# schmeing/ReSeq

Hardware: AMD Instinct MI355X
Metric: simulated read-pairs/sec (2x150 bp) (higher is better)
Workload: dtype f64

## Files before the change

### reseq_amd/csrc/rsq_core.h

```cpp
#pragma once
#include "rsq_types.h"
#if !defined(__HIPCC_RTC__)
#include <math.h>
#endif

namespace rsq {

struct Words {
    uint32_t w0, w1, w2, w3;
};


RSQ_HD Words philox(uint64_t seed, uint32_t c0, uint32_t c1, uint32_t c2, uint32_t c3) {
    uint32_t k0 = (uint32_t)seed, k1 = (uint32_t)(seed >> 32);
#pragma unroll
    for (int r = 0; r < 10; ++r) {
        const uint64_t p0 = (uint64_t)0xD2511F53u * c0, p1 = (uint64_t)0xCD9E8D57u * c2;
        const uint32_t hi0 = (uint32_t)(p0 >> 32), lo0 = (uint32_t)p0, hi1 = (uint32_t)(p1 >> 32), lo1 = (uint32_t)p1;
        c0 = hi1 ^ c1 ^ k0;
        c1 = lo1;
        c2 = hi0 ^ c3 ^ k1;
        c3 = lo0;
        k0 += 0x9E3779B9u;
        k1 += 0xBB67AE85u;
// ... 269 lines not shown
template <int NM, class Par0>
RSQ_HD uint32_t draw(const DevTable &t, const double *__restrict__ pool, Par0 par0, const uint32_t (&idx)[NM], double u, double &prob_sum) {
    prob_sum = 0.0;
    if (!t.k) return 0;
    const uint32_t kp = row_stride(t.k);
    GlobalRow m[NM];
#pragma unroll
    for (int n = 0; n < NM; ++n) m[n].p = pool + t.off[n] + (size_t)clamp_row(t, n, idx[n]) * kp;
    uint32_t col;
    if constexpr (NM == 3) col = draw_rows_k(t.k, u, prob_sum, m[0], m[1], m[2]);
    else col = draw_rows_k(t.k, u, prob_sum, m[0], m[1], m[2], m[3]);
    return par0[t.par0_off + col];
}

template <int NM, class Par0>
RSQ_HD uint32_t draw_slim(const DevTable &t, const double *__restrict__ pool, Par0 par0, const uint32_t (&idx)[NM], double u, double &prob_sum) {
    prob_sum = 0.0;
    if (!t.k) return 0;
    const uint32_t kp = row_stride(t.k);
    GlobalRow m[NM];
#pragma unroll
    for (int n = 0; n < NM; ++n) m[n].p = pool + t.off[n] + (size_t)clamp_row(t, n, idx[n]) * kp;
    uint32_t col;
    if constexpr (NM == 3) col = draw_rows<1>(t.k, u, prob_sum, m[0], m[1], m[2]);
    else col = draw_rows<1>(t.k, u, prob_sum, m[0], m[1], m[2], m[3]);
    return par0[t.par0_off + col];
}

struct GlobalTables {
    using Sum = double;
    const DevSim &S;
    RSQ_HD const DevTable &quality(uint32_t i) const { return S.quality[i]; }
    RSQ_HD const DevTable &seq_quality(uint32_t i) const { return S.seq_quality[i]; }
    RSQ_HD uint32_t draw_quality(uint32_t i, const uint32_t (&idx)[4], uint32_t word, double &ps) const { return draw<4>(S.quality[i], S.pool, S.par0, idx, u32_to_unit(word), ps); }
    RSQ_HD uint32_t draw_base_call(uint32_t i, const uint32_t (&idx)[4], uint32_t word, double &ps) const { return draw<4>(S.base_call[i], S.pool, S.par0, idx, u32_to_unit(word), ps); }
    RSQ_HD uint32_t draw_indel(uint32_t i, const uint32_t (&idx)[3], uint32_t word, double &ps) const { return draw<3>(S.indels[i], S.pool, S.par0, idx, u32_to_unit(word), ps); }
    RSQ_HD uint32_t draw_seq_quality(uint32_t i, const uint32_t (&idx)[3], uint32_t word, double &ps) const { return draw<3>(S.seq_quality[i], S.pool, S.par0, idx, u32_to_unit(word), ps); }
};

RSQ_HD uint32_t ref_base(const uint64_t *__restrict__ words, uint64_t word_off, uint32_t pos) {
    return (uint32_t)(words[word_off + (pos >> 5)] >> ((pos & 31u) * 2u)) & 3u;
}
RSQ_HD uint32_t ref_gc_count(const uint64_t *__restrict__ words, uint64_t word_off, uint32_t a, uint32_t b) {
    uint32_t gc = 0;
    const uint64_t kLow = 0x5555555555555555ull;
    for (uint32_t w = a >> 5; w <= ((b - 1) >> 5) && a < b; ++w) {
        uint64_t x = words[word_off + w];
        uint64_t g = (x ^ (x >> 1)) & kLow;
        uint32_t lo = w == (a >> 5) ? (a & 31u) : 0u;
        uint32_t hi = w == ((b - 1) >> 5) ? ((b - 1) & 31u) + 1u : 32u;
        if (lo) g &= ~0ull << (2u * lo);
        if (hi < 32u) g &= (1ull << (2u * hi)) - 1ull;
#if defined(__HIP_DEVICE_COMPILE__)
        gc += (uint32_t)__popcll(g);
#else
        gc += (uint32_t)__builtin_popcountll(g);
#endif
    }
    return gc;
}

RSQ_HD uint32_t gc_low(uint64_t x, uint32_t n_bases) {
    const uint64_t g = (x ^ (x >> 1)) & 0x5555555555555555ull & ((1ull << (2u * n_bases)) - 1ull);
#if defined(__HIP_DEVICE_COMPILE__)
    return (uint32_t)__popcll(g);
#else
    return (uint32_t)__builtin_popcountll(g);
#endif
// ... 135 lines not shown
    uint32_t seq_qual, qual, error_rate, num_errors;
    uint32_t last_written_qual;
    uint32_t iteration;
};

RSQ_HD uint32_t draw_read_length(const DevSim &S, uint32_t seg, uint32_t fragment_length, double u) {
    const DevReadLengths &rl = S.read_lengths[seg];
    if (rl.fixed) return rl.fixed;
    const double random_value = u * (double)S.insert_lengths[fragment_length];
    double counter = 0.0;
    const uint32_t row = fragment_length - rl.row_first;
    const uint32_t from = rl.row_from[row] & 0xFFFFu;
    uint32_t read_len = (from + (rl.row_ptr[row + 1] - rl.row_ptr[row])) & 0xFFFFu;
    while (counter <= random_value) {
        const bool more = read_len > from;
        read_len = (read_len - 1u) & 0xFFFFu;
        if (!more) break;
        counter += (double)rl.values[rl.row_ptr[row] + (read_len - from)];
    }
    return read_len;
}

template <class Src>
RSQ_HD void template_totals_loop(const Src &src, uint32_t n, uint32_t &gc, uint32_t &rate_sum) {
    for (uint32_t k = 0; k < n; ++k) {
        if (is_gc(src.base(k))) ++gc;
        rate_sum += src.sys_base(k) >> 8;
    }
}

struct AdapterSrc {
    const uint8_t *seq;
    const uint16_t *sys_;
    RSQ_HD uint32_t base(uint32_t k) const { return seq[k]; }
    RSQ_HD uint32_t sys_base(uint32_t k) const { return sys_[k]; }
    RSQ_HD uint32_t sys_deleted(uint32_t k) const { return sys_[k]; }
};

struct ReadMachine {
    enum : uint32_t { kTemplate = 0, kAdapter = 1, kTail = 2, kDone = 3 };
    FillState par;
    CigarRun cg;
    uint32_t phase, seg, tile_id, tbase;
    uint32_t org_pos, org_len;
    uint32_t adapter_id, adapter_a0;
    uint32_t iter_m, hard_clip, tail_length, pos_tail, n_indels;
    uint32_t start_cut_word;

    RSQ_HD void idle() {
        par = FillState{};
        cg = CigarRun{'M', 0, 0};
        phase = kDone;
        seg = tile_id = tbase = org_pos = org_len = adapter_id = adapter_a0 = iter_m = hard_clip = tail_length = pos_tail = n_indels = start_cut_word = 0;
    }
    template <class Tab, class Src>
    RSQ_HD void init(const DevSim &S, const Tab &tab, const Stream &st, uint32_t seg_, uint32_t tile, uint32_t fragment_length, const Src &src) {
        seg = seg_;
        tile_id = tile;
        tbase = (seg * RSQ_SIM(S, n_tiles) + tile_id) * 4u;
        par.read_pos = 0;
        par.previous_indel_type = 0;
        par.indel_pos = 0;
        par.base_call = 5;
        par.gc_seq = 0;
        par.qual = 1;
        par.error_rate = 0;
// ... 63 lines not shown
                org_pos = adapter_pos;
                tail_length = discrete_draw(S.polya_cp, S.polya_n, u32_to_unit(h1.w0)) + S.polya_from;
                cg.element = 'S';
                cg.length = 0;
                phase = kAdapter;
            } else if (phase == kAdapter) {
                if (par.read_pos < par.read_length && org_pos < org_len) return true;
                if (cg.length) cg.flush();
                if (!(par.read_pos < par.read_length)) {
                    phase = kDone;
                    return false;
                }
                hard_clip = par.read_length - par.read_pos;
                cg.chars += digits10(hard_clip) + 1u;
                pos_tail = 0;
                phase = kTail;
            } else if (phase == kTail) {
                if (par.read_pos < par.read_length) return true;
                phase = kDone;
                return false;
            } else return false;
        }
    }

    template <class Tab, class Src, class Out>
    RSQ_HD bool step(const DevSim &S, const Tab &tab, const Stream &st, const Src &src, Out &out) {
        if (!advance(S, st)) return false;
        iterate(S, tab, st, src, out);
        return true;
    }
    RSQ_HD bool in_template() const { return phase == kTemplate && par.read_pos < par.read_length && org_pos < org_len; }
    template <bool TEMPLATE_PART = false, class Tab, class Src, class Out>
    RSQ_HD void iterate(const DevSim &S, const Tab &tab, const Stream &st, const Src &src, Out &out) {
        const bool tail = !TEMPLATE_PART && phase == kTail, from_template = TEMPLATE_PART || phase == kTemplate;
        const DevAdapters &ad = S.adapters[seg];
        const uint32_t it = par.iteration;
        const Words w = st.step(2u + it);
        typename Tab::Sum prob_sum;
        uint32_t indel = 0, org_base = 0;
        if (!tail) {
            const uint32_t idx_i[3] = {par.indel_pos, par.read_pos, par.gc_seq};
            indel = tab.draw_indel(par.previous_indel_type * 6u + par.base_call, idx_i, w.w0, prob_sum);
            if (0 == prob_sum) indel = 0;
            org_base = from_template ? src.base(org_pos) : (uint32_t)ad.seqs[adapter_a0 + org_pos];
        }
        const uint32_t qi = tbase + org_base;
        const bool regular = !tail && 0 == indel, deletion = !tail && 1 == indel;
        uint32_t dom_error = 0;
        if (regular) {
            const uint32_t se = from_template ? src.sys_base(org_pos) : (uint32_t)ad.sys[adapter_a0 + org_pos];
            dom_error = se & 0xFFu;
            par.error_rate = se >> 8;
        } else if (deletion) {
            par.error_rate = (from_template ? src.sys_deleted(org_pos) : (uint32_t)ad.sys[adapter_a0 + org_pos]) >> 8;
        }
        uint32_t q = 0;
        if (!deletion) {
            const uint32_t idx_q[4] = {par.seq_qual, par.qual, par.read_pos, par.error_rate};
            q = tab.draw_quality(qi, idx_q, w.w1, prob_sum);
            if (0 == prob_sum) {
                if (regular) q = par.read_pos ? par.last_written_qual : tab.quality(qi).max_value;
                else if (tail) q = par.read_pos ? par.last_written_qual : q;
                else q = par.qual;
            }
        }
        uint32_t put_base = 0, op_code = 0;
// ... 15 lines not shown
            par.qual = q;
            put_base = pos_tail < tail_length ? 0u : discrete_draw(S.overrun_cp, 4, u32_to_unit(w.w3));
            ++pos_tail;
        } else {
            put_base = indel - 2u;
            op_code = 2u;
            element = 'I';
        }
        if (element) {
            const uint32_t is_indel = deletion || insertion ? 1u : 0u;
            n_indels += is_indel;
            par.num_errors += is_indel;
            if (element == cg.element) {
                ++cg.length;
                par.indel_pos += is_indel;
            } else {
                cg.flush();
                cg.element = element;
                cg.length = 1;
                par.indel_pos = is_indel;
                par.previous_indel_type = deletion ? 1u : 0u;
            }
            if (!insertion) ++org_pos;
        }
        if (!deletion) {
            out.put(par.read_pos, put_base, q + RSQ_SIM(S, phred_offset));
            par.last_written_qual = q;
            ++par.read_pos;
        }
        if (!tail) out.op(it, op_code);
        par.iteration = it + 1u;
    }

    RSQ_HD void finalize(ReadMeta &meta) const {
        meta.read_len = (uint16_t)par.read_length;
        meta.num_errors = (uint16_t)par.num_errors;
        meta.n_iter_m = (uint16_t)iter_m;
        meta.n_iter_s = (uint16_t)(par.iteration - iter_m - hard_clip);
        meta.hard_clip = (uint16_t)hard_clip;
        meta.tile_id = (uint16_t)tile_id;
        meta.cigar_chars = (uint16_t)cg.chars;
        meta.plain = n_indels ? 0u : 1u;
    }
};

template <class Tab, class Src, class Out>
RSQ_HD void fill_read(const DevSim &S, const Tab &tab, const Stream &st, uint32_t seg, uint32_t tile_id, uint32_t fragment_length, const Src &src, Out &out,
                      ReadMeta &meta) {
    ReadMachine m;
    m.init(S, tab, st, seg, tile_id, fragment_length, src);
    while (m.step(S, tab, st, src, out)) {}
    m.finalize(meta);
}

}
```

### reseq_amd/csrc/rsq_reads.h

```cpp
#pragma once
#include "rsq_core.h"
#include "rsq_variants.h"
#include "rsq_text.h"

namespace rsq {

struct ReadOut {
    WordColumn seq, qual, ops;
    uint32_t cur_word, cur_index;
    uint32_t seq_word, qual_word, n_put;
    RSQ_HD void put(uint32_t pos, uint32_t base, uint32_t qual_char) {
        const uint32_t sh = (pos & 3u) * 8u;
        seq_word |= base << sh;
        qual_word |= qual_char << sh;
        n_put = pos + 1u;
        if ((pos & 3u) == 3u) {
            seq.at(pos >> 2) = seq_word;
            qual.at(pos >> 2) = qual_word;
            seq_word = qual_word = 0;
        }
    }
    RSQ_HD void op(uint32_t it, uint32_t code) {
        const uint32_t wi = it >> 4;
        if (wi != cur_index) {
            ops.at(cur_index) = cur_word;
            cur_word = 0;
            cur_index = wi;
        }
        cur_word |= code << ((it & 15u) * 2u);
    }
    RSQ_HD void finish() {
        ops.at(cur_index) = cur_word;
        if (n_put & 3u) {
            seq.at(n_put >> 2) = seq_word;
            qual.at(n_put >> 2) = qual_word;
        }
    }
};
RSQ_HD ReadOut make_read_out(const WordColumn &seq, const WordColumn &qual, const WordColumn &ops) { return ReadOut{seq, qual, ops, 0u, 0u, 0u, 0u, 0u}; }

struct RawLayout {
    uint32_t *seq, *qual;
    uint32_t *ops;
    ReadMeta *meta;
    uint64_t pitch;
    uint64_t *templates;
    uint32_t template_words;
    const uint32_t *order;
    RSQ_HD uint64_t item_of(uint64_t row) const { return order ? order[row] : row; }
    RSQ_HD WordColumn seq_of(uint64_t r) const { return WordColumn{seq + r, pitch}; }
    RSQ_HD WordColumn qual_of(uint64_t r) const { return WordColumn{qual + r, pitch}; }
    RSQ_HD WordColumn ops_of(uint64_t r) const { return WordColumn{ops + r, pitch}; }
    RSQ_HD ReadOut out_of(uint64_t r) const { return make_read_out(seq_of(r), qual_of(r), ops_of(r)); }
};

struct FragmentSrc {
    const uint64_t *words;
    uint64_t word_off;
    uint32_t first;
    uint32_t len;
    bool reverse;
    const uint16_t *sys_;
    const uint64_t *converted;
    const uint32_t *gc_prefix;
    mutable uint32_t held_word = 0xFFFFFFFFu, held_sys = 0xFFFFFFFFu;
    mutable uint64_t word = 0, sys4 = 0;
    RSQ_HD uint64_t template_word(const uint64_t *from, uint32_t index) const {
        if (index != held_word) {
            held_word = index;
            word = from[index];
        }
        return word;
    }
    RSQ_HD uint32_t org_len() const { return len; }
    RSQ_HD uint32_t ref(uint32_t k) const {
        const uint32_t pos = reverse ? first - 1u - k : first + k, b = (uint32_t)(template_word(words + word_off, pos >> 5) >> ((pos & 31u) * 2u)) & 3u;
        return reverse ? 3u - b : b;
    }
    RSQ_HD uint32_t base(uint32_t k) const { return converted ? (uint32_t)(template_word(converted, k >> 5) >> ((k & 31u) * 2u)) & 3u : ref(k); }
    RSQ_HD uint32_t sys_base(uint32_t k) const {
        if ((k >> 2) != held_sys) {
            held_sys = k >> 2;
#if defined(__HIP_DEVICE_COMPILE__)
            sys4 = *reinterpret_cast<const uint64_t __attribute__((aligned(2))) *>(sys_ + (k & ~3u));
#else
            memcpy(&sys4, sys_ + (k & ~3u), 8);
#endif
        }
        return (uint32_t)(sys4 >> ((k & 3u) * 16u)) & 0xFFFFu;
    }
    RSQ_HD uint32_t sys_deleted(uint32_t k) const { return sys_base(k); }
    RSQ_HD void totals(uint32_t n, uint32_t &gc, uint32_t &rate_sum) const {
        if (!converted && !gc_prefix) return template_totals_loop(*this, n, gc, rate_sum);
        if (converted) gc += ref_gc_count(converted, 0, 0, n);
        else gc += reverse ? ref_gc_count_prefix(words, gc_prefix, word_off, first - n, first) : ref_gc_count_prefix(words, gc_prefix, word_off, first, first + n);
        rate_sum += rate_total(n);
    }
// ... 138 lines not shown
                        ++t;
                        continue;
                    }
                    left = side.len(var);
                }
            }
            uint32_t run;
            if (left) {
                run = left < length - t ? left : length - t;
                left -= run;
                if (!left) {
                    var = side.next(var);
                    ++x;
                }
            } else {
                int64_t until = out;
                if (side.variant(var) && side.at(var) > x && side.at(var) < until) until = side.at(var);
                run = until - x < (int64_t)(length - t) ? (uint32_t)(until - x) : length - t;
                x += run;
            }
            ct_convert_run(tmpl, t, run, rate, d);
            t = (uint16_t)(t + run);
        }
        region = side.next(region);
        if (side.region(region) && side.entry(region) > x) skip_to(region);
    }
}
RSQ_HD void ct_conversion(uint64_t *tmpl, uint32_t length, const MethView &m, const VarView *r, uint32_t allele, uint32_t start_pos, bool reversed, VarStart from, MethDraws &d) {
    if (reversed) methylation_walk<true>(tmpl, length, m, r, allele, start_pos, from, d);
    else methylation_walk<false>(tmpl, length, m, r, allele, start_pos, from, d);
}

struct EmptySrc {
    RSQ_HD void totals(uint32_t, uint32_t &, uint32_t &) const {}
    RSQ_HD uint32_t org_len() const { return 0; }
    RSQ_HD uint32_t base(uint32_t) const { return 0; }
    RSQ_HD uint32_t sys_base(uint32_t) const { return 0; }
    RSQ_HD uint32_t sys_deleted(uint32_t) const { return 0; }
};

RSQ_HD uint32_t draw_tile(const DevSim &S, uint32_t c0, uint32_t c1, uint32_t c2, uint32_t c3base) {
    if (RSQ_SIM(S, n_tiles) > 1) return discrete_draw(S.tile_cp, RSQ_SIM(S, n_tiles), u32_to_unit(philox(S.seed, c0, c1, c2, c3base).w0));
    return 0;
}

RSQ_HD uint32_t lds_desc_count(uint32_t n_tiles) { return 25u * n_tiles + 12u; }
RSQ_HD uint32_t image_qbase(const DevSim &S, uint32_t seg, uint32_t first_tile) { return (seg * RSQ_SIM(S, n_tiles) + first_tile) * 4u; }
constexpr uint32_t kDescWords = sizeof(DevTable) / 4u;

#if defined(__HIP_DEVICE_COMPILE__)
#define RSQ_NOINLINE __device__ __noinline__
#else
#define RSQ_NOINLINE inline
#endif
#if defined(RSQ_SCREEN_STATS) && !defined(__HIP_DEVICE_COMPILE__)
#define RSQ_SCREEN_COUNT(family, decided) (++RSQ_SCREEN_STATS[family][0], RSQ_SCREEN_STATS[family][1] += !(decided))
#else
#define RSQ_SCREEN_COUNT(family, decided) ((void)0)
#endif

template <int NM>
#if defined(__HIP_DEVICE_COMPILE__)
__device__ __noinline__
#else
inline
#endif
// ... 11 lines not shown

#define RSQ_GEO_ROW(S, fam, n, v) ((uint32_t)geo_clamp((int32_t)(v) - (int32_t)RSQ_PLAN(S, fam.from[n]), (int32_t)RSQ_PLAN(S, fam.last[n])))
RSQ_HD int32_t geo_clamp(int32_t d, int32_t last) {
#if defined(__clang__)
    return __builtin_elementwise_min(__builtin_elementwise_max(d, 0), last);
#else
    return d < 0 ? 0 : (d > last ? last : d);
#endif
}

template <uint32_t MASK>
struct ScreenTables {
    using Sum = uint32_t;
    static constexpr int QQ = (int)MASK;
    const DevSim &S;
    const RSQ_LDS float *img;
    uint32_t qbase;
    const RSQ_LDS float *ring_;
    uint32_t t;
    uint32_t demand = 0xFFFFFFFFu;
    RSQ_HD DevTable desc(uint32_t local) const { return reinterpret_cast<const RSQ_LDS DevTable *>(img)[local]; }
    RSQ_HD uint32_t par0_at() const { return RSQ_PLAN(S, desc_words) - RSQ_PLAN(S, par0_words); }
    RSQ_HD DevTable quality(uint32_t i) const { return desc(i - qbase); }
    RSQ_HD DevTable seq_quality(uint32_t i) const { return desc(24u * RSQ_PLAN(S, img_tiles) + 12u + i - qbase / 4u); }
    RSQ_HD const RSQ_LDS float *ring(uint32_t p) const { return ring_ + (p % kRingSlots) * RSQ_PLAN(S, ring_stride); }
    RSQ_HD bool in_ring(uint32_t p) const { return t - p <= kRingLag; }
    template <int NM>
    RSQ_HD uint32_t exact(uint32_t desc, const uint32_t (&idx)[NM], uint32_t word, uint32_t &ps) const {
        const uint32_t r = exact_draw_call<NM>(S.pool, img, par0_at(), desc, idx[0], idx[1], idx[2], NM == 4 ? idx[NM - 1] : 0u, word);
        ps = (r >> 31) ^ 1u;
        return r & 0x7FFFFFFFu;
    }
    template <int NM>
    RSQ_HD uint32_t settle(bool decided, uint32_t values, uint32_t column, uint32_t desc, const uint32_t (&idx)[NM], uint32_t u, uint32_t &ps) const {
        uint32_t value = reinterpret_cast<const RSQ_LDS uint8_t *>(img)[values + column];
        ps = 1u;
        decided = decided && !RSQ_SIM(S, force_exact);
        if (!decided) value = exact<NM>(desc, idx, u, ps);
        return value;
    }

    RSQ_HD uint32_t draw_quality(uint32_t i, const uint32_t (&idx)[4], uint32_t u, uint32_t &ps) const {
        const uint32_t local = i - qbase, slot = RSQ_PLAN(S, slot_q), nr = RSQ_PLAN(S, rate_rows_q), r3 = RSQ_GEO_ROW(S, q, 3, idx[3]);
        const RSQ_LDS float *mine = img + RSQ_PLAN(S, q.lds) + local * RSQ_PLAN(S, q.lds_stride);
        const LdsRow32 m0{mine + RSQ_GEO_ROW(S, q, 0, idx[0]) * slot}, m1{mine + (RSQ_PLAN(S, q.before[1]) + RSQ_GEO_ROW(S, q, 1, idx[1])) * slot};
        const bool near = in_ring(idx[2]);
        const LdsRow32 m2{ring_ + (near ? idx[2] % kRingSlots : kRingSlots) * RSQ_PLAN(S, ring_stride) + local * slot};
        const LdsRow32 m3{img + RSQ_PLAN(S, q3_off) + local * RSQ_PLAN(S, q3_stride) + (r3 < nr ? r3 : 0u) * slot};
        uint32_t col = 0;
        const bool decided = draw_screened<QQ>(u, col, m0, m1, m2, m3) && (near || idx[2] == demand) && r3 < nr;
        RSQ_SCREEN_COUNT(0, decided);
        return settle<4>(decided, RSQ_PLAN(S, q.values), local * slot + col, local, idx, u, ps);
    }
    RSQ_HD uint32_t draw_base_call(uint32_t i, const uint32_t (&idx)[4], uint32_t u, uint32_t &ps) const {
        const uint32_t local = i - qbase * 5u, slot = RSQ_PLAN(S, slot_b), nr = RSQ_PLAN(S, rate_rows_b), r3 = RSQ_GEO_ROW(S, b, 3, idx[3]);
        const uint32_t g = 4u * (RSQ_PLAN(S, b.off32) + i * (RSQ_PLAN(S, b.table_rows) * slot));
        const LdsRow32 m0{img + RSQ_PLAN(S, b.lds) + local * RSQ_PLAN(S, b.lds_stride) + RSQ_GEO_ROW(S, b, 0, idx[0]) * slot};
        const PoolRow32 m1{S.pool32, g + 4u * (RSQ_PLAN(S, b.before[1]) + RSQ_GEO_ROW(S, b, 1, idx[1])) * slot};
        const uint32_t r2 = RSQ_GEO_ROW(S, b, 2, idx[2]);
        const bool m2_staged = RSQ_PLAN(S, b.lds2) != kNoLds, staged = r3 < nr;
        const MixedRow32 m2{LdsRow32{img + (m2_staged ? RSQ_PLAN(S, b.lds2) + local * RSQ_PLAN(S, b.lds2_stride) + r2 * slot : 0u)},
                            PoolRow32{S.pool32, g + 4u * (RSQ_PLAN(S, b.before[2]) + r2) * slot}, m2_staged};
        const MixedRow32 m3{LdsRow32{img + RSQ_PLAN(S, b3_off) + local * RSQ_PLAN(S, b3_stride) + (staged ? r3 : 0u) * slot}, PoolRow32{S.pool32, g + 4u * (RSQ_PLAN(S, b.before[3]) + r3) * slot}, staged};
        uint32_t col = 0;
        const bool decided = draw_screened<(int)kQuadsSmall>(u, col, m0, m1, m2, m3);
        RSQ_SCREEN_COUNT(1, decided);
        return settle<4>(decided, RSQ_PLAN(S, b.values), local * slot + col, 4u * RSQ_PLAN(S, img_tiles) + local, idx, u, ps);
    }
    RSQ_HD uint32_t draw_indel(uint32_t i, const uint32_t (&idx)[3], uint32_t u, uint32_t &ps) const {
        const RSQ_LDS DevTable *d = reinterpret_cast<const RSQ_LDS DevTable *>(img) + (24u * RSQ_PLAN(S, img_tiles) + i);
        const uint32_t range = d->sure_range, lo16 = range & 0xFFFFu;
        const bool sure = (u >> 16) - lo16 < (range >> 16) - lo16 && idx[0] <= d->from[0];
        RSQ_SCREEN_COUNT(3, sure);
        ps = 1u;
        if (sure) return 0;
        const uint32_t slot = RSQ_PLAN(S, slot_i), r0 = RSQ_GEO_ROW(S, i, 0, idx[0]);
        const uint32_t g = 4u * (RSQ_PLAN(S, i.off32) + i * (RSQ_PLAN(S, i.table_rows) * slot));
        const bool m0_staged = RSQ_PLAN(S, i.lds) != kNoLds;
        const MixedRow32 m0{LdsRow32{img + (m0_staged ? RSQ_PLAN(S, i.lds) + i * RSQ_PLAN(S, i.lds_stride) + r0 * slot : 0u)}, PoolRow32{S.pool32, g + 4u * r0 * slot}, m0_staged};
        const PoolRow32 m1{S.pool32, g + 4u * (RSQ_PLAN(S, i.before[1]) + RSQ_GEO_ROW(S, i, 1, idx[1])) * slot}, m2{S.pool32, g + 4u * (RSQ_PLAN(S, i.before[2]) + RSQ_GEO_ROW(S, i, 2, idx[2])) * slot};
        uint32_t col = 0;
        const bool decided = draw_screened<(int)kQuadsSmall>(u, col, m0, m1, m2);
        RSQ_SCREEN_COUNT(2, decided);
        return settle<3>(decided, RSQ_PLAN(S, i.values), i * slot + col, 24u * RSQ_PLAN(S, img_tiles) + i, idx, u, ps);
    }
    RSQ_HD uint32_t draw_seq_quality(uint32_t i, const uint32_t (&idx)[3], uint32_t u, uint32_t &ps) const {
        const uint32_t r = exact_draw_call<3>(S.pool, img, par0_at(), 24u * RSQ_PLAN(S, img_tiles) + 12u + i - qbase / 4u, idx[0], idx[1], idx[2], 0u, u);
        ps = (r >> 31) ^ 1u;
        return r & 0x7FFFFFFFu;
    }
};

RSQ_HD void lds_stage_descriptors(const DevSim &S, RSQ_LDS float *img, uint32_t qbase, uint32_t tid, uint32_t nthreads) {
    const uint32_t T = RSQ_PLAN(S, img_tiles);
    RSQ_LDS uint32_t *dst = reinterpret_cast<RSQ_LDS uint32_t *>(img);
    const uint32_t wq = 4u * T * kDescWords, wb = 20u * T * kDescWords, wi = 12u * kDescWords, ws = T * kDescWords;
    const uint32_t *q = reinterpret_cast<const uint32_t *>(S.quality + qbase), *b = reinterpret_cast<const uint32_t *>(S.base_call + qbase * 5u),
                   *in = reinterpret_cast<const uint32_t *>(S.indels), *sq = reinterpret_cast<const uint32_t *>(S.seq_quality + qbase / 4u);
    const uint32_t tiles_at = S.quality[qbase].par0_off, shift = tiles_at - RSQ_PLAN(S, par0_indel_bytes);
    for (uint32_t i = tid; i < wq; i += nthreads) dst[i] = q[i] - (i % kDescWords == 1u ? shift : 0u);
// ... 42 lines not shown
    const uint32_t table = item / RSQ_PLAN(S, quads_q), c = item % RSQ_PLAN(S, quads_q), slot = RSQ_PLAN(S, slot_q);
    return RingItem{4u * (RSQ_PLAN(S, q.off32) + ((qbase + table) * RSQ_PLAN(S, q.table_rows) + RSQ_PLAN(S, q.before[2])) * slot + 4u * c), table * slot + 4u * c};
}
RSQ_HD Quad lds_ring_load(const DevSim &S, const RingItem &it, uint32_t p) { return PoolRow32{S.pool32, it.rows + 4u * RSQ_GEO_ROW(S, q, 2, p) * RSQ_PLAN(S, slot_q)}.quad(0u); }
RSQ_HD void lds_ring_store(const DevSim &S, const RingItem &it, RSQ_LDS float *ring, uint32_t p, const Quad &q) {
    *reinterpret_cast<RSQ_LDS Quad *>(ring + (p % kRingSlots) * RSQ_PLAN(S, ring_stride) + it.at) = q;
}
RSQ_HD void lds_ring_stage(const DevSim &S, const RingItem &it, RSQ_LDS float *ring, uint32_t p) { lds_ring_store(S, it, ring, p, lds_ring_load(S, it, p)); }
RSQ_HD void lds_ring_stage_demand(const DevSim &S, const RingItem &it, RSQ_LDS float *ring, uint32_t p) {
    *reinterpret_cast<RSQ_LDS Quad *>(ring + kRingSlots * RSQ_PLAN(S, ring_stride) + it.at) = lds_ring_load(S, it, p);
}
RSQ_HD void lds_ring_stage(const DevSim &S, uint32_t qbase, RSQ_LDS float *ring, uint32_t p, uint32_t item) { lds_ring_stage(S, lds_ring_item(S, qbase, item), ring, p); }
RSQ_HD FragmentSrc fragment_src(const DevSim &S, const Fragment &f, uint32_t seg, uint32_t end) {
    const uint32_t L = S.seq_len[f.seq];
    const uint32_t want = S.read_lengths[seg].to + RSQ_SIM(S, max_len_deletion);
    FragmentSrc src;
    src.words = hap_words(S, f.allele);
    src.word_off = S.seq_word_off[f.seq];
    src.len = f.len < want ? f.len : want;
    src.reverse = seg != f.strand;
    src.first = src.reverse ? end : f.start;
    src.sys_ = src.reverse ? S.sys_rev + S.seq_base_off[f.seq] + (L - end) : S.sys_fwd + S.seq_base_off[f.seq] + f.start;
    src.converted = nullptr;
    src.gc_prefix = hap_gc_prefix(S, f.allele);
    return src;
}
RSQ_HD FragmentSrc fragment_src(const DevSim &S, const Fragment &f, uint32_t seg) { return fragment_src(S, f, seg, f.start + f.len); }

struct VariantSrc : FragmentSrc {
    const DevVariant *var;
    const uint16_t *err;
    uint32_t n_var, L, allele;
    uint32_t *walk_error;
    uint32_t spos0, cur0, var_pos0;
    mutable uint32_t spos, cur, var_pos;
    RSQ_HD const DevVariant &var_at(uint32_t i) const { return reverse ? var[n_var - 1u - i] : var[i]; }
    RSQ_HD uint32_t var_spos(uint32_t i) const { return reverse ? L - 1u - var_at(i).pos : var_at(i).pos; }
    RSQ_HD uint32_t var_err(uint32_t i, uint32_t k) const { return err[var_at(i).off + k]; }
    RSQ_HD uint32_t lower_bound(uint32_t sp) const {
        uint32_t lo = 0, hi = n_var;
        while (lo < hi) {
            const uint32_t mid = (lo + hi) >> 1;
            if (var_spos(mid) < sp) lo = mid + 1u;
            else hi = mid;
        }
        return lo;
    }
    RSQ_HD uint32_t seek(uint32_t sp) const {
        uint32_t c = cur < n_var ? cur : n_var;
        while (c > 0u && var_spos(c - 1u) >= sp) --c;
        while (c < n_var && var_spos(c) < sp) ++c;
        return c;
    }
    RSQ_HD uint32_t block_end(uint32_t sp) const { return reverse ? L - ((L - sp - 1u) / kBlockSize) * kBlockSize : (sp / kBlockSize + 1u) * kBlockSize; }
    mutable uint32_t vs_cur, bend_cur;
    mutable uint32_t quiet_until;
    RSQ_HD void refresh() const {
        vs_cur = cur < n_var ? var_spos(cur) : 0xFFFFFFFFu;
        bend_cur = block_end(spos);
        uint32_t q = bend_cur - 1u;
        if (vs_cur < q) q = vs_cur;
        if (L < q) q = L;
        quiet_until = var_pos ? 0u : q;
    }
    RSQ_HD void rewind() const {
        spos = spos0;
// ... 131 lines not shown
    const VarStart from = reversed ? VarStart{fv.end_var, fv.end_var_pos} : VarStart{fv.start_var, fv.start_var_pos};
    const uint32_t at = reversed ? fv.end : f.start;
    allele_template(allele_view(S, f.seq, f.allele), at, from, tl, reversed, tmpl, template_words);
    if (S.meth_ptr) {
        const MethView m = meth_view(S, f.seq, f.allele);
        MethDraws d{S.seed, f.start, f.seq | (fv.sub << 22), f.len, (kDomMethylation << 28) | ((reversed ? 1u : 0u) << 27) | ((uint32_t)f.allele << 17), 0xFFFFFFFFu,
                    Words{0, 0, 0, 0}};
        ct_conversion(tmpl, tl, m, &r, f.allele, at, reversed, from, d);
    }
}

template <class Tab>
RSQ_HD void fill_fragment_read(const DevSim &S, const Tab &tab, const Fragment &f, uint32_t seg, ReadOut &out, ReadMeta &meta) {
    const uint32_t c2 = f.len | ((uint32_t)f.dup << 16);
    const uint32_t tile = draw_tile(S, f.start, f.seq, c2, pair_c3(kDomPair, f.strand, 2, f.allele));
    const Stream st{S.seed, f.start, f.seq, c2, pair_c3(kDomPair, f.strand, seg, f.allele)};
    if (S.variants_loaded) fill_read(S, tab, st, seg, tile, f.len, variant_src(S, f, nullptr, seg), out, meta);
    else fill_read(S, tab, st, seg, tile, f.len, fragment_src(S, f, seg), out, meta);
}
template <class Tab>
RSQ_HD void fill_adapter_only_read(const DevSim &S, const Tab &tab, uint64_t i, uint32_t seg, ReadOut &out, ReadMeta &meta) {
    const uint32_t tile = draw_tile(S, (uint32_t)i, 0xFFFFFFFFu, (uint32_t)(i >> 32), pair_c3(kDomPair, 0, 2));
    const Stream st{S.seed, (uint32_t)i, 0xFFFFFFFFu, (uint32_t)(i >> 32), pair_c3(kDomPair, 0, seg)};
    fill_read(S, tab, st, seg, tile, 0u, EmptySrc{}, out, meta);
}

struct RecordSrc {
    const uint8_t *seq;
    const uint8_t *dom, *rate;
    uint32_t len;
    uint32_t safe;
    mutable uint32_t group;
    mutable uint64_t w_seq, w_dom, w_rate;
    RSQ_HD static uint64_t load8(const uint8_t *p, uint32_t off, uint32_t safe) {
        uint64_t w = 0;
        if (off + 8u <= safe) {
#if defined(__HIP_DEVICE_COMPILE__)
            w = *reinterpret_cast<const uint64_t __attribute__((aligned(1))) *>(p + off);
#else
            memcpy(&w, p + off, 8);
#endif
        } else {
            for (uint32_t j = 0; j < 8u && off + j < safe; ++j) w |= (uint64_t)p[off + j] << (8u * j);
        }
        return w;
    }
    RSQ_HD void hold(uint32_t k) const {
        const uint32_t g = k >> 3;
        if (g == group) return;
        group = g;
        w_seq = load8(seq, g * 8u, safe);
        w_dom = load8(dom, g * 8u, safe);
        w_rate = load8(rate, g * 8u, safe);
    }
    RSQ_HD uint32_t org_len() const { return len; }
    RSQ_HD uint32_t base(uint32_t k) const {
        hold(k);
        return (uint32_t)(w_seq >> ((k & 7u) * 8u)) & 0xFFu;
    }
    RSQ_HD uint32_t sys_base(uint32_t k) const {
        hold(k);
        const uint32_t sh = (k & 7u) * 8u;
        return ((uint32_t)(w_dom >> sh) & 0xFFu) | (((uint32_t)(w_rate >> sh) & 0xFFu) << 8);
    }
    RSQ_HD uint32_t sys_deleted(uint32_t k) const { return sys_base(k); }
    RSQ_HD void totals(uint32_t n, uint32_t &gc, uint32_t &rate_sum) const {
        const uint64_t kOnes = 0x0101010101010101ull, kEven = 0x00FF00FF00FF00FFull;
        for (uint32_t g = (n + 7u) >> 3; g--;) {
            hold(g * 8u);
            const uint32_t left = n - g * 8u;
            const uint64_t keep = left >= 8u ? ~0ull : (1ull << (8u * left)) - 1ull;
            const uint64_t w = w_seq & keep, r = w_rate & keep;
            const uint64_t high = (w >> 2) | (w >> 3) | (w >> 4) | (w >> 5) | (w >> 6) | (w >> 7);
            const uint64_t is = (w ^ (w >> 1)) & ~high & kOnes;
            gc += (uint32_t)((is * kOnes) >> 56);
            const uint64_t pairs = (r & kEven) + ((r >> 8) & kEven);
            rate_sum += (uint32_t)((pairs * 0x0001000100010001ull) >> 48);
        }
    }
};
RSQ_HD RecordSrc record_src(const uint8_t *seqs, const uint8_t *dom, const uint8_t *rate, uint32_t read_len, uint64_t i, uint64_t n) {
    const uint64_t rest = (n - i) * read_len;
    return RecordSrc{seqs + i * read_len, dom + i * read_len, rate + i * read_len, read_len, rest > 0xFFFFFFFFull ? 0xFFFFFFFFu : (uint32_t)rest, 0xFFFFFFFFu, 0, 0, 0};
}
RSQ_HD RecordSrc record_src_at(const uint8_t *seqs, const uint8_t *dom, const uint8_t *rate, uint32_t at, uint32_t len, uint32_t bytes) {
    return RecordSrc{seqs + at, dom + at, rate + at, len, bytes - at, 0xFFFFFFFFu, 0, 0, 0};
}
struct PackedRecordSrc {
    const uint16_t *codes;
    uint32_t len;
    uint32_t safe;
    mutable uint32_t group;
    mutable uint64_t lo, hi;
    RSQ_HD void hold(uint32_t k) const {
        const uint32_t g = k >> 3;
        if (g == group) return;
        group = g;
        const uint16_t *p = codes + 8u * g;
        if (8u * g + 8u <= safe) {
#if defined(__HIP_DEVICE_COMPILE__)
            lo = *reinterpret_cast<const uint64_t __attribute__((aligned(2))) *>(p);
            hi = *reinterpret_cast<const uint64_t __attribute__((aligned(2))) *>(p + 4);
#else
            memcpy(&lo, p, 8);
            memcpy(&hi, p + 4, 8);
#endif
        } else {
            lo = hi = 0;
            for (uint32_t j = 0; j < 8u && 8u * g + j < safe; ++j) (j < 4u ? lo : hi) |= (uint64_t)p[j] << (16u * (j & 3u));
        }
    }
    RSQ_HD uint32_t half(uint32_t k) const {
        hold(k);
        return (uint32_t)(((k & 4u) ? hi : lo) >> (16u * (k & 3u))) & 0xFFFFu;
    }
    RSQ_HD uint32_t org_len() const { return len; }
    RSQ_HD uint32_t base(uint32_t k) const { return half(k) & 3u; }
    RSQ_HD uint32_t sys_base(uint32_t k) const {
        const uint32_t h = half(k);
        return ((h >> 2) & 7u) | (h & 0xFF00u);
    }
    RSQ_HD uint32_t sys_deleted(uint32_t k) const { return sys_base(k); }
    RSQ_HD void totals(uint32_t n, uint32_t &gc, uint32_t &rate_sum) const {
        const uint64_t kHalfOnes = 0x0001000100010001ull;
        for (uint32_t g = (n + 7u) >> 3; g--;) {
            hold(g * 8u);
// ... 46 lines not shown
    return PairStream{(uint32_t)adapter_only_number, 0xFFFFFFFFu, (uint32_t)(adapter_only_number >> 32), 0u};
}

#if RSQ_DEVICE_BUILD
template <uint32_t MASK>
__device__ RSQ_LDS float *fill_stage_image(const DevSim &S, float *lds_image, uint32_t qbase) {
    RSQ_LDS float *img = (RSQ_LDS float *)lds_image;
    if (MASK) {
        lds_stage_descriptors(S, img, qbase, threadIdx.x, blockDim.x);
        __syncthreads();
        lds_stage_rows(S, img, qbase, threadIdx.x, blockDim.x);
        __syncthreads();
    }
    return img;
}
template <uint32_t MASK, class Src>
__device__ void fill_wave_reads(const DevSim &S, RSQ_LDS float *img, uint32_t qbase, uint32_t seg, bool active, const Stream &st, uint32_t tile, uint32_t fragment_length,
                                const Src &src, ReadOut &out, ReadMeta &meta) {
    ReadMachine m;
    if constexpr (MASK == 0) {
        const GlobalTables tab{S};
        if (active) {
            m.init(S, tab, st, seg, tile, fragment_length, src);
            while (m.step(S, tab, st, src, out)) {}
        }
    } else {
        const uint32_t lane = threadIdx.x & 63u, n_items = lds_ring_items(S);
        RSQ_LDS float *ring = img + RSQ_PLAN(S, ring_off) + (threadIdx.x >> 6) * kRingRows * RSQ_PLAN(S, ring_stride);
        ScreenTables<MASK> tab{S, img, qbase, ring, 0u};
        m.idle();
        if (active) m.init(S, tab, st, seg, tile, fragment_length, src);
        const RingItem mine = lds_ring_item(S, qbase, lane < n_items ? lane : 0u);
        Quad ahead = lane < n_items ? lds_ring_load(S, mine, 0u) : zero_quad();
        auto begin_step = [&](uint32_t t) {
            if (lane < n_items) {
                lds_ring_store(S, mine, ring, t, ahead);
                ahead = lds_ring_load(S, mine, t + 1u);
            }
            for (uint32_t item = lane + 64u; item < n_items; item += 64u) lds_ring_stage(S, qbase, ring, t, item);
            __builtin_amdgcn_wave_barrier();
            tab.t = t;
            const uint64_t lagging = __builtin_amdgcn_ballot_w64(m.phase != ReadMachine::kDone && t - m.par.read_pos > kRingLag);
            tab.demand = 0xFFFFFFFFu;
            if (lagging) {
                const uint32_t p = __builtin_amdgcn_readlane(m.par.read_pos, __builtin_ctzll(lagging));
                if (lane < n_items) lds_ring_stage_demand(S, mine, ring, p);
                for (uint32_t item = lane + 64u; item < n_items; item += 64u) lds_ring_stage_demand(S, lds_ring_item(S, qbase, item), ring, p);
                __builtin_amdgcn_wave_barrier();
                tab.demand = p;
            }
        };
        uint32_t t = 0;
        for (; !RSQ_ANY(!m.in_template()); ++t) {
            begin_step(t);
            m.template iterate<true>(S, tab, st, src, out);
            __builtin_amdgcn_wave_barrier();
        }
        for (; RSQ_ANY(m.phase != ReadMachine::kDone); ++t) {
            begin_step(t);
            m.step(S, tab, st, src, out);
            __builtin_amdgcn_wave_barrier();
        }
    }
    if (active) {
        m.finalize(meta);
        out.finish();
    }
}

template <uint32_t MASK, class Chunk>
__device__ void fill_binned_loop(const DevSim &S, float *lds_image, const FillBins &bins, Chunk &&chunk) {
    RSQ_LDS float *img = (RSQ_LDS float *)lds_image;
    RSQ_LDS uint32_t *sched = reinterpret_cast<RSQ_LDS uint32_t *>(img + (MASK ? RSQ_PLAN(S, total_words) : 0u));
    const uint32_t lane = threadIdx.x & 63u;
    if (threadIdx.x == 0) sched[1] = 0xFFFFFFFFu;
    for (bool first_choice = true;; first_choice = false) {
        if (threadIdx.x < 64u) {
            uint64_t best = 0;
            if (first_choice) {
                const uint64_t total = bins.chunk_ptr[bins.n_bins], target = ((2u * (uint64_t)blockIdx.x + 1u) * total) / (2u * gridDim.x);
                uint32_t lo = 0, hi = bins.n_bins;
                while (hi - lo > 1u) {
                    const uint32_t mid = (lo + hi) >> 1;
                    if (bins.chunk_ptr[mid] <= target) lo = mid;
                    else hi = mid;
                }
                best = total ? ((uint64_t)1 << 32) | (0xFFFFFFFFu - lo) : 0u;
            } else {
                for (uint32_t b = lane; b < bins.n_bins; b += 64u) {
                    const uint32_t n = (bins.bin_count[b] + 63u) / 64u, done = __hip_atomic_load(&bins.next_chunk[b], __ATOMIC_RELAXED, __HIP_MEMORY_SCOPE_AGENT),
                                   on_it = __hip_atomic_load(&bins.workers[b], __ATOMIC_RELAXED, __HIP_MEMORY_SCOPE_AGENT), left = done < n ? n - done : 0u;
                    const uint64_t score = (uint64_t)left * 4096u / (on_it + 1u), packed = (score << 32) | (0xFFFFFFFFu - b);
// ... 172 lines not shown
```

Measured before the change: 242.7 million.

## Add branchless template-phase iterate with skip flags for unneeded table draws

Adds a dedicated iterate_template path used during the wave-synchronous template phase. It computes the indel, quality and base-call draws with select-style logic instead of divergent branches. A 'needed' flag lets the quality and base-call draws skip the exact fallback and screen counting when the result is discarded. The lag ballot also drops the phase check while every lane is known to be running. The aim is less wave divergence and fewer exact table lookups per iteration, at the cost of a duplicated code path that must stay in sync with the generic one.

```diff
diff --git a/reseq_amd/csrc/rsq_core.h b/reseq_amd/csrc/rsq_core.h
--- a/reseq_amd/csrc/rsq_core.h
+++ b/reseq_amd/csrc/rsq_core.h
@@ -325,8 +325,12 @@
     const DevSim &S;
     RSQ_HD const DevTable &quality(uint32_t i) const { return S.quality[i]; }
     RSQ_HD const DevTable &seq_quality(uint32_t i) const { return S.seq_quality[i]; }
-    RSQ_HD uint32_t draw_quality(uint32_t i, const uint32_t (&idx)[4], uint32_t word, double &ps) const { return draw<4>(S.quality[i], S.pool, S.par0, idx, u32_to_unit(word), ps); }
-    RSQ_HD uint32_t draw_base_call(uint32_t i, const uint32_t (&idx)[4], uint32_t word, double &ps) const { return draw<4>(S.base_call[i], S.pool, S.par0, idx, u32_to_unit(word), ps); }
+    RSQ_HD uint32_t draw_quality(uint32_t i, const uint32_t (&idx)[4], uint32_t word, double &ps, bool needed = true) const {
+        return needed ? draw<4>(S.quality[i], S.pool, S.par0, idx, u32_to_unit(word), ps) : (ps = 1.0, 0u);
+    }
+    RSQ_HD uint32_t draw_base_call(uint32_t i, const uint32_t (&idx)[4], uint32_t word, double &ps, bool needed = true) const {
+        return needed ? draw<4>(S.base_call[i], S.pool, S.par0, idx, u32_to_unit(word), ps) : (ps = 1.0, 0u);
+    }
     RSQ_HD uint32_t draw_indel(uint32_t i, const uint32_t (&idx)[3], uint32_t word, double &ps) const { return draw<3>(S.indels[i], S.pool, S.par0, idx, u32_to_unit(word), ps); }
     RSQ_HD uint32_t draw_seq_quality(uint32_t i, const uint32_t (&idx)[3], uint32_t word, double &ps) const { return draw<3>(S.seq_quality[i], S.pool, S.par0, idx, u32_to_unit(word), ps); }
 };
@@ -528,6 +532,7 @@
 struct AdapterSrc {
     const uint8_t *seq;
     const uint16_t *sys_;
+    static constexpr bool kSysIsLookup = true;
     RSQ_HD uint32_t base(uint32_t k) const { return seq[k]; }
     RSQ_HD uint32_t sys_base(uint32_t k) const { return sys_[k]; }
     RSQ_HD uint32_t sys_deleted(uint32_t k) const { return sys_[k]; }
@@ -657,6 +662,7 @@
     RSQ_HD bool in_template() const { return phase == kTemplate && par.read_pos < par.read_length && org_pos < org_len; }
     template <bool TEMPLATE_PART = false, class Tab, class Src, class Out>
     RSQ_HD void iterate(const DevSim &S, const Tab &tab, const Stream &st, const Src &src, Out &out) {
+        if constexpr (TEMPLATE_PART) return iterate_template(S, tab, st, src, out);
         const bool tail = !TEMPLATE_PART && phase == kTail, from_template = TEMPLATE_PART || phase == kTemplate;
         const DevAdapters &ad = S.adapters[seg];
         const uint32_t it = par.iteration;
@@ -738,6 +744,53 @@
         par.iteration = it + 1u;
     }
 
+    template <class Tab, class Src, class Out>
+    RSQ_HD void iterate_template(const DevSim &S, const Tab &tab, const Stream &st, const Src &src, Out &out) {
+        const uint32_t it = par.iteration;
+        const Words w = st.step(2u + it);
+        typename Tab::Sum prob_sum;
+        const uint32_t idx_i[3] = {par.indel_pos, par.read_pos, par.gc_seq};
+        uint32_t indel = tab.draw_indel(par.previous_indel_type * 6u + par.base_call, idx_i, w.w0, prob_sum);
+        indel = 0 == prob_sum ? 0u : indel;
+        const bool regular = 0 == indel, deletion = 1 == indel, insertion = indel > 1u;
+        const uint32_t org_base = src.base(org_pos), qi = tbase + org_base, is_indel = regular ? 0u : 1u;
+        uint32_t se;
+        if constexpr (Src::kSysIsLookup) se = src.sys_base(org_pos);
+        else {
+            se = par.error_rate << 8;
+            if (regular) se = src.sys_base(org_pos);
+            else if (deletion) se = src.sys_deleted(org_pos);
+        }
+        par.error_rate = insertion ? par.error_rate : se >> 8;
+        const uint32_t idx_q[4] = {par.seq_qual, par.qual, par.read_pos, par.error_rate};
+        uint32_t q = tab.draw_quality(qi, idx_q, w.w1, prob_sum, !deletion);
+        if (0 == prob_sum) q = regular ? (par.read_pos ? par.last_written_qual : tab.quality(qi).max_value) : par.qual;
+        const uint32_t idx_b[4] = {q, par.read_pos, par.num_errors, par.error_rate};
+        uint32_t call = tab.draw_base_call(qi * 5u + (se & 0xFFu), idx_b, w.w2, prob_sum, regular);
+        call = 0 == prob_sum ? org_base : call;
+        par.qual = regular ? q : par.qual;
+        par.base_call = regular ? call : par.base_call;
+        par.num_errors += (regular && call != org_base ? 1u : 0u) + is_indel;
+        n_indels += is_indel;
+        out.put_if(!deletion, par.read_pos, regular ? call : indel - 2u, q + RSQ_SIM(S, phred_offset));
+        out.op(it, indel < 2u ? indel : 2u);
+        par.last_written_qual = deletion ? par.last_written_qual : q;
+        par.read_pos += deletion ? 0u : 1u;
+        org_pos += insertion ? 0u : 1u;
+        par.iteration = it + 1u;
+        const char element = regular ? 'M' : (deletion ? 'D' : 'I');
+        const uint32_t run = cg.length;
+        ++cg.length;
+        par.indel_pos += is_indel;
+        if (element != cg.element) {
+            cg.chars += digits10(run) + 1u;
+            cg.element = element;
+            cg.length = 1;
+            par.indel_pos = is_indel;
+            par.previous_indel_type = deletion ? 1u : 0u;
+        }
+    }
+
     RSQ_HD void finalize(ReadMeta &meta) const {
         meta.read_len = (uint16_t)par.read_length;
         meta.num_errors = (uint16_t)par.num_errors;
diff --git a/reseq_amd/csrc/rsq_reads.h b/reseq_amd/csrc/rsq_reads.h
--- a/reseq_amd/csrc/rsq_reads.h
+++ b/reseq_amd/csrc/rsq_reads.h
@@ -20,6 +20,17 @@
             seq_word = qual_word = 0;
         }
     }
+    RSQ_HD void put_if(bool keep, uint32_t pos, uint32_t base, uint32_t qual_char) {
+        const uint32_t sh = (pos & 3u) * 8u;
+        seq_word |= (keep ? base : 0u) << sh;
+        qual_word |= (keep ? qual_char : 0u) << sh;
+        n_put = pos + (keep ? 1u : 0u);
+        if (keep && (pos & 3u) == 3u) {
+            seq.at(pos >> 2) = seq_word;
+            qual.at(pos >> 2) = qual_word;
+            seq_word = qual_word = 0;
+        }
+    }
     RSQ_HD void op(uint32_t it, uint32_t code) {
         const uint32_t wi = it >> 4;
         if (wi != cur_index) {
@@ -63,6 +74,7 @@
     const uint16_t *sys_;
     const uint64_t *converted;
     const uint32_t *gc_prefix;
+    static constexpr bool kSysIsLookup = true;
     mutable uint32_t held_word = 0xFFFFFFFFu, held_sys = 0xFFFFFFFFu;
     mutable uint64_t word = 0, sys4 = 0;
     RSQ_HD uint64_t template_word(const uint64_t *from, uint32_t index) const {
@@ -267,6 +279,7 @@
 }
 
 struct EmptySrc {
+    static constexpr bool kSysIsLookup = true;
     RSQ_HD void totals(uint32_t, uint32_t &, uint32_t &) const {}
     RSQ_HD uint32_t org_len() const { return 0; }
     RSQ_HD uint32_t base(uint32_t) const { return 0; }
@@ -344,15 +357,15 @@
         return r & 0x7FFFFFFFu;
     }
     template <int NM>
-    RSQ_HD uint32_t settle(bool decided, uint32_t values, uint32_t column, uint32_t desc, const uint32_t (&idx)[NM], uint32_t u, uint32_t &ps) const {
+    RSQ_HD uint32_t settle(bool decided, uint32_t values, uint32_t column, uint32_t desc, const uint32_t (&idx)[NM], uint32_t u, uint32_t &ps, bool needed = true) const {
         uint32_t value = reinterpret_cast<const RSQ_LDS uint8_t *>(img)[values + column];
         ps = 1u;
-        decided = decided && !RSQ_SIM(S, force_exact);
+        decided = (decided && !RSQ_SIM(S, force_exact)) || !needed;
         if (!decided) value = exact<NM>(desc, idx, u, ps);
         return value;
     }
 
-    RSQ_HD uint32_t draw_quality(uint32_t i, const uint32_t (&idx)[4], uint32_t u, uint32_t &ps) const {
+    RSQ_HD uint32_t draw_quality(uint32_t i, const uint32_t (&idx)[4], uint32_t u, uint32_t &ps, bool needed = true) const {
         const uint32_t local = i - qbase, slot = RSQ_PLAN(S, slot_q), nr = RSQ_PLAN(S, rate_rows_q), r3 = RSQ_GEO_ROW(S, q, 3, idx[3]);
         const RSQ_LDS float *mine = img + RSQ_PLAN(S, q.lds) + local * RSQ_PLAN(S, q.lds_stride);
         const LdsRow32 m0{mine + RSQ_GEO_ROW(S, q, 0, idx[0]) * slot}, m1{mine + (RSQ_PLAN(S, q.before[1]) + RSQ_GEO_ROW(S, q, 1, idx[1])) * slot};
@@ -361,10 +374,10 @@
         const LdsRow32 m3{img + RSQ_PLAN(S, q3_off) + local * RSQ_PLAN(S, q3_stride) + (r3 < nr ? r3 : 0u) * slot};
         uint32_t col = 0;
         const bool decided = draw_screened<QQ>(u, col, m0, m1, m2, m3) && (near || idx[2] == demand) && r3 < nr;
-        RSQ_SCREEN_COUNT(0, decided);
-        return settle<4>(decided, RSQ_PLAN(S, q.values), local * slot + col, local, idx, u, ps);
-    }
-    RSQ_HD uint32_t draw_base_call(uint32_t i, const uint32_t (&idx)[4], uint32_t u, uint32_t &ps) const {
+        if (needed) RSQ_SCREEN_COUNT(0, decided);
+        return settle<4>(decided, RSQ_PLAN(S, q.values), local * slot + col, local, idx, u, ps, needed);
+    }
+    RSQ_HD uint32_t draw_base_call(uint32_t i, const uint32_t (&idx)[4], uint32_t u, uint32_t &ps, bool needed = true) const {
         const uint32_t local = i - qbase * 5u, slot = RSQ_PLAN(S, slot_b), nr = RSQ_PLAN(S, rate_rows_b), r3 = RSQ_GEO_ROW(S, b, 3, idx[3]);
         const uint32_t g = 4u * (RSQ_PLAN(S, b.off32) + i * (RSQ_PLAN(S, b.table_rows) * slot));
         const LdsRow32 m0{img + RSQ_PLAN(S, b.lds) + local * RSQ_PLAN(S, b.lds_stride) + RSQ_GEO_ROW(S, b, 0, idx[0]) * slot};
@@ -376,8 +389,8 @@
         const MixedRow32 m3{LdsRow32{img + RSQ_PLAN(S, b3_off) + local * RSQ_PLAN(S, b3_stride) + (staged ? r3 : 0u) * slot}, PoolRow32{S.pool32, g + 4u * (RSQ_PLAN(S, b.before[3]) + r3) * slot}, staged};
         uint32_t col = 0;
         const bool decided = draw_screened<(int)kQuadsSmall>(u, col, m0, m1, m2, m3);
-        RSQ_SCREEN_COUNT(1, decided);
-        return settle<4>(decided, RSQ_PLAN(S, b.values), local * slot + col, 4u * RSQ_PLAN(S, img_tiles) + local, idx, u, ps);
+        if (needed) RSQ_SCREEN_COUNT(1, decided);
+        return settle<4>(decided, RSQ_PLAN(S, b.values), local * slot + col, 4u * RSQ_PLAN(S, img_tiles) + local, idx, u, ps, needed);
     }
     RSQ_HD uint32_t draw_indel(uint32_t i, const uint32_t (&idx)[3], uint32_t u, uint32_t &ps) const {
         const RSQ_LDS DevTable *d = reinterpret_cast<const RSQ_LDS DevTable *>(img) + (24u * RSQ_PLAN(S, img_tiles) + i);
@@ -486,6 +499,7 @@
     const uint16_t *err;
     uint32_t n_var, L, allele;
     uint32_t *walk_error;
+    static constexpr bool kSysIsLookup = false;
     uint32_t spos0, cur0, var_pos0;
     mutable uint32_t spos, cur, var_pos;
     RSQ_HD const DevVariant &var_at(uint32_t i) const { return reverse ? var[n_var - 1u - i] : var[i]; }
@@ -683,6 +697,7 @@
     uint32_t safe;
     mutable uint32_t group;
     mutable uint64_t w_seq, w_dom, w_rate;
+    static constexpr bool kSysIsLookup = true;
     RSQ_HD static uint64_t load8(const uint8_t *p, uint32_t off, uint32_t safe) {
         uint64_t w = 0;
         if (off + 8u <= safe) {
@@ -743,6 +758,7 @@
     uint32_t safe;
     mutable uint32_t group;
     mutable uint64_t lo, hi;
+    static constexpr bool kSysIsLookup = true;
     RSQ_HD void hold(uint32_t k) const {
         const uint32_t g = k >> 3;
         if (g == group) return;
@@ -855,7 +871,7 @@
         if (active) m.init(S, tab, st, seg, tile, fragment_length, src);
         const RingItem mine = lds_ring_item(S, qbase, lane < n_items ? lane : 0u);
         Quad ahead = lane < n_items ? lds_ring_load(S, mine, 0u) : zero_quad();
-        auto begin_step = [&](uint32_t t) {
+        auto begin_step = [&](uint32_t t, bool all_running) {
             if (lane < n_items) {
                 lds_ring_store(S, mine, ring, t, ahead);
                 ahead = lds_ring_load(S, mine, t + 1u);
@@ -863,7 +879,8 @@
             for (uint32_t item = lane + 64u; item < n_items; item += 64u) lds_ring_stage(S, qbase, ring, t, item);
             __builtin_amdgcn_wave_barrier();
             tab.t = t;
-            const uint64_t lagging = __builtin_amdgcn_ballot_w64(m.phase != ReadMachine::kDone && t - m.par.read_pos > kRingLag);
+            const uint64_t lagging = all_running ? __builtin_amdgcn_ballot_w64(t - m.par.read_pos > kRingLag)
+                                                 : __builtin_amdgcn_ballot_w64(m.phase != ReadMachine::kDone && t - m.par.read_pos > kRingLag);
             tab.demand = 0xFFFFFFFFu;
             if (lagging) {
                 const uint32_t p = __builtin_amdgcn_readlane(m.par.read_pos, __builtin_ctzll(lagging));
@@ -875,12 +892,12 @@
         };
         uint32_t t = 0;
         for (; !RSQ_ANY(!m.in_template()); ++t) {
-            begin_step(t);
+            begin_step(t, true);
             m.template iterate<true>(S, tab, st, src, out);
             __builtin_amdgcn_wave_barrier();
         }
         for (; RSQ_ANY(m.phase != ReadMachine::kDone); ++t) {
-            begin_step(t);
+            begin_step(t, false);
             m.step(S, tab, st, src, out);
             __builtin_amdgcn_wave_barrier();
         }
```

After: 244.6 million, median of 6. No clear change (+0.8%).
